# Ji4chenLi/t2v-turbo

Measured on AMD Instinct MI355X. Metric: UNet denoise steps/sec (16f 320x512 latent), higher is better.
Workload: dtype bf16; 1 GPU; VideoCrafter2 UNet forward, B=1 per GPU, latent (1,4,16,40,64), ctx (1,77,1024), 4-step LCM timestep table, random-init weights (zero-init tensors re-drawn); parallelism=replicas x1, hip_graph=True, graph_captured=True

## Files before the change

### t2v-turbo_amd/csrc/build.py

```python
import os
import subprocess
import sys

HERE = os.path.dirname(os.path.abspath(__file__))
PKG = os.path.dirname(HERE)
ROOT = os.path.dirname(PKG)
SOURCES = ["gemm.hip", "gemm_exp.hip", "gemm_fuse.hip", "conv_halo.hip", "linear_pr.hip", "norm.hip", "attention.hip", "elementwise.hip", "backward.hip", "backward_unet.hip", "train.hip", "attention_bwd.hip", "wgrad_tn.hip", "full_grad.hip", "replay.hip"]
EXPERIMENTAL = os.environ.get("T2V_EXPERIMENTAL") == "1"
if EXPERIMENTAL:
    SOURCES = SOURCES + ["gemm2.hip", "ffn.hip"]
LIB = os.path.abspath(os.environ["T2V_HIP_LIB_OUT"]) if os.environ.get("T2V_HIP_LIB_OUT") else os.path.join(PKG, "libt2v_hip_exp.so" if EXPERIMENTAL else "libt2v_hip.so")
FLAGS = ["--offload-arch=gfx950", "-O3", "-std=c++17", "-fPIC", "-Wno-unused-value",
         "-I", os.path.join(ROOT, "include"), "-I", HERE] + (["-DT2V_EXPERIMENTAL"] if EXPERIMENTAL else []) + os.environ.get("T2V_EXTRA_HIPCC_FLAGS", "").split()


def _hipcc():
    for c in (os.environ.get("HIPCC"), "/opt/rocm/bin/hipcc", "hipcc"):
        if c and (os.path.isabs(c) and os.path.exists(c) or not os.path.isabs(c)):
            return c
    return "hipcc"


def needs_build():
    if not os.path.exists(LIB):
        return True
    t = os.path.getmtime(LIB)
    deps = [os.path.join(HERE, s) for s in SOURCES] + [os.path.join(HERE, "common.h"), os.path.join(HERE, "gn_bwd_common.h"), os.path.join(HERE, "tile80.h"), os.path.join(HERE, "gemm2.h"), os.path.join(HERE, "gelu_poly.h"),
                                                        os.path.join(ROOT, "include", "t2v_hip.h")]
    return any(os.path.getmtime(d) > t for d in deps)


EXTRA_DEPS = {"gemm.hip": ["gemm2.h", "gelu_poly.h"], "gemm_exp.hip": ["gemm.hip", "gemm2.h", "gelu_poly.h"], "gemm_fuse.hip": ["gemm.hip", "gemm2.h", "gelu_poly.h"],
              "linear_pr.hip": ["gelu_poly.h"],
              "conv_halo.hip": ["tile80.h"], "gemm2.hip": ["tile80.h", "gemm2.h"], "backward.hip": ["gn_bwd_common.h"],
              "backward_unet.hip": ["gn_bwd_common.h"]}


def _stale(src, obj):
    if not os.path.exists(obj):
        return True
    t = os.path.getmtime(obj)
    deps = [os.path.join(HERE, src), os.path.join(HERE, "common.h"), os.path.join(ROOT, "include", "t2v_hip.h"), os.path.abspath(__file__)]
    deps += [os.path.join(HERE, d) for d in EXTRA_DEPS.get(src, [])]
    return any(os.path.getmtime(d) > t for d in deps)


def build(force=False, verbose=True):
    if not force and not needs_build():
        return LIB
    hipcc = _hipcc()
    objs = []
    procs = []
    for s in SOURCES:
        variant = bool(os.environ.get("T2V_HIP_LIB_OUT") or os.environ.get("T2V_EXTRA_HIPCC_FLAGS") or EXPERIMENTAL)
        o = os.path.join(HERE, s.replace(".hip", ".variant.o" if variant else ".o"))
        objs.append(o)
        if not force and not variant and not _stale(s, o):
            continue
        cmd = [hipcc] + FLAGS + ["-c", os.path.join(HERE, s), "-o", o]
        if verbose:
            print(" ".join(cmd), flush=True)
        procs.append((cmd, subprocess.Popen(cmd)))
    for cmd, p in procs:
        if p.wait() != 0:
            raise RuntimeError("hipcc failed: " + " ".join(cmd))
    cmd = [hipcc, "--offload-arch=gfx950", "-shared", "-fPIC", "-o", LIB] + objs
    if verbose:
        print(" ".join(cmd), flush=True)
    subprocess.check_call(cmd)
    return LIB


if __name__ == "__main__":
    build(force="--force" in sys.argv)
    print(LIB)
```

### t2v-turbo_amd/csrc/gemm.hip

```cpp
#include "common.h"
#ifdef T2V_EXPERIMENTAL
#include "gemm2.h"
#endif
#include "gelu_poly.h"
#include <cstdlib>
#include <type_traits>

struct GemmParams {
    t2v_gemm_desc d;
    const void* zero;
    int K, nk, taps, nsrc;
    int gh, gw;
    int kh, kw, stride, pad_y, pad_x, ups;
    int h_out, w_out;
    int tiles_m, tiles_n;
    int xcd_m, xcd_n;
    int nblk;
    int blk_start[8], blk_r0[8], blk_c0[8], blk_w[8];
    int vec4;
    int splits, nk_per_split;
    float* ws;
    int debug;
};

// ... 1009 lines not shown
}

}

int t2v_gemm_launch_experimental(int cfg, GemmParams& p, hipStream_t s);
int t2v_gemm_launch_ln(int cfg, GemmParams& p, hipStream_t s);
int t2v_gemm_launch_fused(int cfg, int fuse, GemmParams& p, hipStream_t s);
int t2v_gemm_fuse_tile(int cfg, int act, int fuse);
#ifdef T2V_GEMM_FUSE_ONLY
namespace {
template <int BM, int BN, int WM, int WN, int STAGES, int BK, int WPE>
int launch_fused(int fuse, GemmParams& p, hipStream_t s) {
    switch (fuse) {
        case 1: return launch_impl<BM, BN, WM, WN, STAGES, BK, WPE, true, false, false, 1>(p, s);
        case 2: return launch_impl<BM, BN, WM, WN, STAGES, BK, WPE, true, false, false, 2>(p, s);
        case 4: return launch_impl<BM, BN, WM, WN, STAGES, BK, WPE, true, false, false, 4>(p, s);
        case 8: return launch_impl<BM, BN, WM, WN, STAGES, BK, WPE, true, false, false, 8>(p, s);
        case 16: return launch_impl<BM, BN, WM, WN, STAGES, BK, WPE, true, false, false, 16>(p, s);
        case 18: return launch_impl<BM, BN, WM, WN, STAGES, BK, WPE, true, false, false, 18>(p, s);
        default: return T2V_EINVAL;
    }
}
}
int t2v_gemm_fuse_tile(int cfg, int act, int fuse) {
    if ((fuse == 4 || (fuse & 16)) && cfg == 19) cfg = 7;
    switch (cfg) {
        case 1: case 4: case 10: case 18: case 26: case 30: case 33: return 4;
        case 31: case 32: return act == T2V_ACT_GEGLU ? 4 : 31;
        case 6: case 7: case 13: case 16: case 19: case 25: return cfg == 19 ? 19 : (cfg == 16 ? 16 : 7);
        case 11: case 14: case 17: case 29: return cfg == 17 ? 17 : 11;
        case 12: case 15: case 20: case 21: case 24: case 27: return cfg == 20 ? 20 : 12;
        case 22: case 23: case 28: return act == T2V_ACT_GEGLU ? 17 : 23;
        case 3: case 9: return 9;
        case 2: case 5: return 5;
        default: return 0;
    }
}
int t2v_gemm_launch_fused(int cfg, int fuse, GemmParams& p, hipStream_t s) {
    switch (cfg) {
        case 4: return launch_fused<128, 128, 2, 2, 3, 64, 1>(fuse, p, s);
        case 5: return launch_fused<128, 64, 2, 2, 3, 64, 1>(fuse, p, s);
        case 7: return launch_fused<256, 128, 4, 2, 3, 64, 2>(fuse, p, s);
        case 9: return launch_fused<256, 64, 4, 2, 3, 64, 2>(fuse, p, s);
        case 11: return launch_fused<128, 256, 2, 4, 3, 64, 2>(fuse, p, s);
        case 12: return launch_fused<256, 256, 2, 4, 2, 64, 2>(fuse, p, s);
        case 16: return launch_fused<256, 128, 2, 2, 3, 32, 2>(fuse, p, s);
        case 17: return launch_fused<128, 256, 1, 4, 3, 32, 2>(fuse, p, s);
        case 19: return launch_fused<256, 128, 4, 2, 3, 32, 4>(fuse, p, s);
        case 20: return launch_fused<256, 256, 2, 4, 4, 32, 2>(fuse, p, s);
        case 23: return launch_fused<160, 320, 5, 2, 3, 32, 3>(fuse, p, s);
        case 31: return launch_fused<128, 128, 2, 4, 3, 64, 2>(fuse, p, s);
        default: return T2V_EINVAL;
    }
}
#elif defined(T2V_GEMM_EXP_ONLY)
int t2v_gemm_launch_ln(int cfg, GemmParams& p, hipStream_t s) {
    (void)cfg;
    return launch_impl<160, 320, 5, 2, 3, 32, 3, true, false, true>(p, s);
}
int t2v_gemm_launch_experimental(int cfg, GemmParams& p, hipStream_t s) {
    switch (cfg) {
        case 24: return launch<256, 256, 2, 2, 3, 32, 1>(p, s);
        case 25: return launch<256, 128, 4, 2, 2, 64, 2, true>(p, s);
        case 26: return launch<128, 128, 2, 2, 2, 64, 2, true>(p, s);
        case 27: return launch<256, 256, 2, 4, 2, 32, 2, true>(p, s);
        case 28: return launch<160, 320, 5, 2, 2, 32, 3, true>(p, s);
        case 29: return launch<128, 256, 1, 4, 2, 32, 2, true>(p, s);
        case 30: return launch<128, 128, 4, 2, 3, 64, 2>(p, s);
        case 31: return launch<128, 128, 2, 4, 3, 64, 2>(p, s);
        case 32: return launch<128, 128, 2, 4, 4, 32, 2>(p, s);
        case 33: return launch<128, 128, 4, 2, 4, 32, 2>(p, s);
        default: return T2V_EINVAL;
    }
}
#else

namespace {
struct TileCfg { int bm, bn, wtn, bk = 64; };
const TileCfg kCfg[] = {{0, 0, 0},      {128, 128, 64}, {128, 64, 32},  {256, 64, 64}, {128, 128, 64},
                        {128, 64, 32},  {256, 128, 64}, {256, 128, 64}, {64, 128, 32}, {256, 64, 32},
                        {128, 128, 64}, {128, 256, 64},
                        {256, 256, 64}, {256, 128, 64}, {128, 256, 64}, {256, 256, 64},
                        {256, 128, 64, 32}, {128, 256, 64, 32}, {128, 128, 64, 32}, {256, 128, 64, 32},
                        {256, 256, 64, 32}, {256, 256, 64, 32},
                        {160, 320, 32, 64}, {160, 320, 32, 32},
                        {256, 256, 128, 32},
                        {256, 128, 64, 64}, {128, 128, 64, 64}, {256, 256, 64, 32}, {160, 320, 32, 32}, {128, 256, 64, 32},
                        {128, 128, 64, 64}, {128, 128, 32, 64}, {128, 128, 32, 32}, {128, 128, 64, 32}};
constexpr int kNumCfg = 33;

int dispatch(int cfg, GemmParams& p, hipStream_t s) {
    switch (cfg) {
        case 1: return launch<128, 128, 2, 2, 2>(p, s);
        case 2: return launch<128, 64, 2, 2, 2>(p, s);
        case 3: return launch<256, 64, 4, 1, 2>(p, s);
        case 4: return launch<128, 128, 2, 2, 3>(p, s);
        case 5: return launch<128, 64, 2, 2, 3>(p, s);
        case 6: return launch<256, 128, 4, 2, 2>(p, s);
        case 7: return launch<256, 128, 4, 2, 3>(p, s);
        case 8: return launch<64, 128, 1, 4, 3>(p, s);
        case 9: return launch<256, 64, 4, 2, 3>(p, s);
        case 10: return launch<128, 128, 2, 2, 4>(p, s);
        case 11: return launch<128, 256, 2, 4, 3>(p, s);
        case 12: return launch<256, 256, 2, 4, 2>(p, s);
        case 13: return launch<256, 128, 2, 2, 2>(p, s);
        case 14: return launch<128, 256, 1, 4, 2>(p, s);
        case 15: return launch<256, 256, 4, 2, 2>(p, s);
        case 16: return launch<256, 128, 2, 2, 3, 32, 2>(p, s);
        case 17: return launch<128, 256, 1, 4, 3, 32, 2>(p, s);
        case 18: return launch<128, 128, 2, 2, 4, 32, 2>(p, s);
        case 19: return launch<256, 128, 4, 2, 3, 32, 4>(p, s);
        case 20: return launch<256, 256, 2, 4, 4, 32, 2>(p, s);
        case 21: return launch<256, 256, 4, 2, 4, 32, 2>(p, s);
        case 22: return launch<160, 320, 5, 2, 2, 64, 3>(p, s);
        case 23: return launch<160, 320, 5, 2, 3, 32, 3>(p, s);
        case 24: case 25: case 26: case 27: case 28: case 29: case 30: case 31: case 32: case 33:
            return t2v_gemm_launch_experimental(cfg, p, s);
        default: return T2V_EINVAL;
    }
}

}

static int g_force_cfg = 0, g_force_split = 0, g_debug = 0;
extern "C" int t2v_gemm_debug(int bits) { g_debug = bits; return T2V_OK; }
extern "C" int t2v_gemm_force_config(int cfg) { g_force_cfg = cfg; return T2V_OK; }
extern "C" int t2v_gemm_force_split(int s) { g_force_split = s; return T2V_OK; }
extern "C" int t2v_gemm_num_configs(void) { return kNumCfg; }

static int gemm_prepare(const t2v_gemm_desc* dd, GemmParams& p, int& cfg_out, int& fuse, int& fuse_cfg, bool& fuse_ok) {
    T2V_REQUIRE(dd && dd->a0 && dd->w && dd->out, T2V_EINVAL, "t2v_gemm: null pointer");
    T2V_REQUIRE(!dd->ln_in && !dd->gn_coef, T2V_EINVAL, "t2v_gemm: ln_in / gn_coef (a norm of the input rows) are t2v_linear_pr's; normalise first or ask t2v_linear_pr_supported");
    p.d = *dd;
    t2v_gemm_desc& d = p.d;
    if (!d.a1) { d.c1 = 0; d.lda1 = 0; }
    if (d.batch <= 0) d.batch = 1;
    if (d.batch_inner <= 0) d.batch_inner = 1;
    T2V_REQUIRE(d.M > 0 && d.N > 0, T2V_EINVAL, "t2v_gemm: empty problem");
    T2V_REQUIRE(d.c0 > 0 && d.c0 % 64 == 0 && d.c1 % 64 == 0, T2V_ESHAPE, "t2v_gemm: channels must be multiples of 64");
    T2V_REQUIRE(d.lda0 % 8 == 0 && d.lda1 % 8 == 0 && d.ldw % 8 == 0, T2V_ESHAPE, "t2v_gemm: lda/ldw must be multiples of 8");
    T2V_REQUIRE(((uintptr_t)d.a0 % 16 == 0) && ((uintptr_t)d.w % 16 == 0) && (!d.a1 || (uintptr_t)d.a1 % 16 == 0), T2V_ESHAPE,
                "t2v_gemm: operands must be 16-byte aligned");
    T2V_REQUIRE(d.a_stride0 % 8 == 0 && d.a_stride1 % 8 == 0 && d.w_stride0 % 8 == 0 && d.w_stride1 % 8 == 0, T2V_ESHAPE,
                "t2v_gemm: batch strides must be multiples of 8");
    T2V_REQUIRE(d.batch <= 65535, T2V_ESHAPE, "t2v_gemm: batch too large");
    if (d.drop_thr)
        T2V_REQUIRE(d.drop_seed && d.act == T2V_ACT_NONE && d.drop_ncols > 0 && d.drop_ncols % 4 == 0 && d.drop_col0 % 4 == 0 &&
                        d.drop_col0 >= 0 && d.drop_col0 + d.N <= d.drop_ncols && d.batch == 1,
                    T2V_EINVAL, "t2v_gemm: dropout epilogue (seed pointer, column geometry in multiples of 4, no activation, no batch)");
    p.nsrc = d.a1 ? 2 : 1;
    p.gh = d.h_in; p.gw = d.w_in;
    p.kh = 3; p.kw = 3; p.stride = 1; p.pad_y = 1; p.pad_x = 1; p.ups = 0;
    int n_grid = d.n_img;
    switch (d.mode) {
        case T2V_GEMM_LINEAR: p.kh = p.kw = 1; p.pad_y = p.pad_x = 0; p.gh = p.gw = 1; n_grid = d.M; break;
        case T2V_GEMM_CONV3X3: break;
        case T2V_GEMM_CONV3X3_S2: p.stride = 2; break;
        case T2V_GEMM_CONV3X3_S2_PAD01: p.stride = 2; p.pad_y = p.pad_x = 0; break;
        case T2V_GEMM_CONV3X3_UP2: p.ups = 1; break;
        case T2V_GEMM_TCONV3:
            T2V_REQUIRE(d.frames > 0 && d.n_img % d.frames == 0, T2V_EINVAL, "t2v_gemm: frames");
            p.kw = 1; p.pad_x = 0; p.gh = d.frames; p.gw = d.h_in * d.w_in; n_grid = d.n_img / d.frames;
            break;
        default: T2V_REQUIRE(false, T2V_EINVAL, "t2v_gemm: bad mode");
    }
    if (d.mode != T2V_GEMM_LINEAR) T2V_REQUIRE(d.n_img > 0 && d.h_in > 0 && d.w_in > 0, T2V_EINVAL, "t2v_gemm: conv geometry");
    p.taps = p.kh * p.kw;
    p.h_out = ((p.gh << p.ups) + 2 * p.pad_y - p.kh) / p.stride + 1;
    p.w_out = ((p.gw << p.ups) + 2 * p.pad_x - p.kw) / p.stride + 1;
    if (d.mode == T2V_GEMM_CONV3X3_S2_PAD01) {
        p.h_out = (p.gh + 1 - 3) / 2 + 1; p.w_out = (p.gw + 1 - 3) / 2 + 1;
    }
    T2V_REQUIRE((long long)d.M == (long long)n_grid * p.h_out * p.w_out, T2V_EINVAL, "t2v_gemm: M does not match the geometry");
    p.K = p.taps * (d.c0 + d.c1);
    p.nk = p.K / 64;
    T2V_REQUIRE(d.ldw >= p.K, T2V_EINVAL, "t2v_gemm: ldw < K");
    if (d.act == T2V_ACT_GEGLU) T2V_REQUIRE(d.N % 128 == 0, T2V_ESHAPE, "t2v_gemm: GEGLU needs N % 128 == 0");
    if (d.rowvec) T2V_REQUIRE(d.rowvec_div > 0, T2V_EINVAL, "t2v_gemm: rowvec_div");
    p.zero = t2v_zero_page();
    T2V_REQUIRE(p.zero, T2V_EHIP, "t2v_gemm: zero page allocation failed");
    const int n_out = d.act == T2V_ACT_GEGLU ? d.N / 2 : d.N;
    p.vec4 = (d.ldo % 8 == 0) && (n_out % 4 == 0) && ((uintptr_t)d.out % 16 == 0) && (d.o_stride0 % 8 == 0) &&
             (d.o_stride1 % 8 == 0) && (!d.residual || (d.ldr % 8 == 0 && (uintptr_t)d.residual % 16 == 0)) &&
             (!d.bias || (uintptr_t)d.bias % 16 == 0) && (!d.rowvec || ((uintptr_t)d.rowvec % 16 == 0 && d.ld_rowvec % 4 == 0));
    if (d.act == T2V_ACT_GEGLU) T2V_REQUIRE(p.vec4, T2V_ESHAPE, "t2v_gemm: GEGLU needs 8-byte aligned rows");

    int cfg = g_force_cfg ? g_force_cfg : d.tile_cfg;
    if (cfg < 0 || cfg > kNumCfg) cfg = 0;
    if (cfg == 0) {
        if (d.N % 128 == 0 || d.N >= 1024) cfg = (d.M >= 8192 && p.nk >= 8) ? 7 : 4;
        else if (d.M >= 8192 && d.N % 64 == 0) cfg = 9;
        else cfg = 5;
    }
    if (d.act == T2V_ACT_GEGLU && kCfg[cfg].wtn < 64) cfg = 4;
    p.nk = p.K / kCfg[cfg].bk;
    int splits = g_force_split ? g_force_split : d.split_k;
    const long long tiles = (long long)((d.M + kCfg[cfg].bm - 1) / kCfg[cfg].bm) * ((d.N + kCfg[cfg].bn - 1) / kCfg[cfg].bn) * d.batch;
    const bool can_split = d.ws && d.act != T2V_ACT_GEGLU && d.N % 4 == 0 && p.vec4;
    if (splits <= 0) {
        splits = 1;
        if (can_split && tiles < 160 && p.K / 64 >= 16) {
            splits = (int)((448 + tiles - 1) / tiles);
            if (splits > p.K / 512) splits = p.K / 512;
            if (splits > 16) splits = 16;
        }
    }
    if (!can_split) splits = 1;
    if (splits > 1 && (long long)splits * d.batch * d.M * d.N * 4 > d.ws_bytes) {
        splits = (int)(d.ws_bytes / ((long long)d.batch * d.M * d.N * 4));
        if (splits < 2) splits = 1;
    }
    if (splits > p.nk) splits = p.nk;
    p.nk_per_split = (p.nk + splits - 1) / splits;
    splits = (p.nk + p.nk_per_split - 1) / p.nk_per_split;
    p.splits = splits;
    p.ws = (float*)d.ws;
    p.debug = g_debug;
    cfg_out = cfg;
    fuse = (d.rowstat_out ? 1 : 0) | (d.colstat_out ? 2 : 0) | (d.lnf_stats ? 4 : 0) | (d.lora_t ? 16 : 0);
    static const bool fast_dropout = !(getenv("T2V_GEMM_FAST_DROPOUT") && getenv("T2V_GEMM_FAST_DROPOUT")[0] == '0');
    const bool auto_drop = !fuse && !d.lora_t && d.drop_thr && fast_dropout && !d.rowvec && d.act == T2V_ACT_NONE && !d.ln_out && d.batch == 1;
    if (auto_drop) fuse = 8;
    fuse_cfg = 0;
    fuse_ok = false;
    if (fuse) {
        T2V_REQUIRE(fuse == 1 || fuse == 2 || fuse == 4 || fuse == 8 || fuse == 16 || fuse == 18, T2V_EINVAL,
                    "t2v_gemm: one of rowstat_out / colstat_out / lnf_stats per launch (lora_t alone or with colstat_out)");
        if (fuse & 16)
            T2V_REQUIRE(d.lora_u && d.lora_n_leaf > 0 && d.lora_n_leaf % 32 == 0 && d.N % d.lora_n_leaf == 0 && d.ld_lora_t % 8 == 0 &&
                            d.ld_lora_u % 8 == 0 && d.ld_lora_u >= 64 && d.ld_lora_t >= 64 * (d.N / d.lora_n_leaf) &&
                            (uintptr_t)d.lora_t % 16 == 0 && (uintptr_t)d.lora_u % 16 == 0 && d.act == T2V_ACT_NONE &&
                            (!d.drop_thr || (d.drop_seed && d.drop_ncols % 4 == 0 && d.drop_col0 % 4 == 0)),
                        T2V_ESHAPE, "t2v_gemm: lora_t: rank-64 rows [M][64 leaves], lora_u [N][64], N a multiple of lora_n_leaf (% 32), no activation");
        T2V_REQUIRE(!d.ln_out && d.batch == 1, T2V_EINVAL, "t2v_gemm: fused statistics: no batch, no LayerNorm second output");
        if (fuse == 1)
            T2V_REQUIRE(d.N % 32 == 0 && d.ld_rowstat >= d.N / 16 && d.ld_rowstat % 4 == 0 && (uintptr_t)d.rowstat_out % 16 == 0 &&
                            d.act == T2V_ACT_NONE, T2V_ESHAPE, "t2v_gemm: rowstat_out needs N % 32 == 0, ld_rowstat >= N / 16 (% 4), no activation");
        if (fuse & 2)
            T2V_REQUIRE(d.M % 32 == 0 && d.N % 2 == 0 && (uintptr_t)d.colstat_out % 16 == 0 && d.act != T2V_ACT_GEGLU, T2V_ESHAPE,
                        "t2v_gemm: colstat_out needs M % 32 == 0");
        if (fuse == 4)
            T2V_REQUIRE(d.mode == T2V_GEMM_LINEAR && !d.a1 && d.lnf_s && d.bias && d.lnf_nblk > 0 && d.lnf_nblk % 2 == 0 && d.lnf_nblk <= 40 &&
                            d.c0 == 32 * d.lnf_nblk && d.lnf_ld >= 2 * d.lnf_nblk && d.lnf_ld % 4 == 0 && (uintptr_t)d.lnf_stats % 16 == 0 &&
                            (uintptr_t)d.lnf_s % 16 == 0 && !d.residual && !d.rowvec && !d.drop_thr && d.act != T2V_ACT_SILU,
                        T2V_ESHAPE, "t2v_gemm: lnf_stats: LINEAR over C = 32 lnf_nblk <= 1280 channels, lnf_s and bias given, no residual / "
                                    "row vector / dropout");
        fuse_cfg = t2v_gemm_fuse_tile(cfg, d.act, fuse);
        fuse_ok = fuse_cfg != 0 && p.splits == 1 && gemm_is_fast(p, fuse == 8 || (fuse & 16) != 0) && !(d.act == T2V_ACT_GEGLU && kCfg[fuse_cfg].wtn < 64);
        if ((fuse & 16) && fuse_cfg != 0 && d.N != d.lora_n_leaf) {
            const int wtn = fuse_cfg == 23 ? 160 : kCfg[fuse_cfg].wtn;
            for (int s = 0; s < d.N && fuse_ok; s += wtn)
                if ((s + wtn - 1 < d.N ? s + wtn - 1 : d.N - 1) / d.lora_n_leaf - s / d.lora_n_leaf > 1) fuse_ok = false;
        }
        if (fuse == 8 && !(fuse_cfg == cfg || cfg == 28 || cfg == 32)) fuse_ok = false;
        if (fuse_ok) { p.nk = p.K / kCfg[fuse_cfg].bk; p.nk_per_split = p.nk; }
        if (fuse == 8 && !fuse_ok) fuse = 0;
        return T2V_OK;
    }
    return T2V_OK;
}

#ifdef T2V_EXPERIMENTAL
static int g_gemm2 = -1;
extern "C" int t2v_gemm2_enable(int on) { g_gemm2 = on ? 1 : 0; return T2V_OK; }
static int gemm2_route(const t2v_gemm_desc* dd, int fuse, Gemm2Params& p2, int& c2) {
    c2 = 0;
    if (g_gemm2 < 0) g_gemm2 = (getenv("T2V_GEMM2") && getenv("T2V_GEMM2")[0] == '1') ? 1 : 0;
    const int want = g_force_cfg ? g_force_cfg : dd->tile_cfg;
    const int forced = (want == 50 || want == 51) ? want - 49 : 0;
    if ((fuse & ~2) || dd->ln_out || !(forced || (g_gemm2 && !g_force_cfg))) return T2V_OK;
    return t2v_gemm2_prepare(dd, p2, forced, c2);
}
#endif

extern "C" int t2v_gemm_fuse_supported(const t2v_gemm_desc* dd) {
    GemmParams p;
    int cfg = 0, fuse = 0, fuse_cfg = 0;
    bool ok = false;
    const int rc = gemm_prepare(dd, p, cfg, fuse, fuse_cfg, ok);
    if (rc != T2V_OK) return rc;
#ifdef T2V_EXPERIMENTAL
    if (fuse == 2) {
        Gemm2Params p2;
        int c2 = 0;
        const int rc2 = gemm2_route(dd, fuse, p2, c2);
        if (rc2 != T2V_OK) return rc2;
        if (c2) return 1;
    }
#endif
    return ((fuse & ~8) && ok) ? 1 : 0;
}

extern "C" int t2v_gemm_plan(const t2v_gemm_desc* dd, int* tile_cfg, int* splits) {
    GemmParams p;
    int cfg = 0, fuse = 0, fuse_cfg = 0;
    bool ok = false;
    const int rc = gemm_prepare(dd, p, cfg, fuse, fuse_cfg, ok);
    if (rc != T2V_OK) return rc;
    if (tile_cfg) *tile_cfg = (fuse && ok) ? fuse_cfg : cfg;
    if (splits) *splits = p.splits;
    return T2V_OK;
}

extern "C" int t2v_gemm(const t2v_gemm_desc* dd, void* stream) {
    GemmParams p;
    int cfg = 0, fuse = 0, fuse_cfg = 0;
    bool fuse_ok = false;
    const int rc = gemm_prepare(dd, p, cfg, fuse, fuse_cfg, fuse_ok);
    if (rc != T2V_OK) return rc;
    t2v_gemm_desc& d = p.d;
    hipStream_t s = (hipStream_t)stream;
#ifdef T2V_EXPERIMENTAL
    {
        Gemm2Params p2;
        int c2 = 0;
        const int rc2 = gemm2_route(dd, fuse, p2, c2);
        if (rc2 != T2V_OK) return rc2;
        if (c2) return t2v_gemm2_dispatch(c2, p2, s);
    }
#endif
    if (fuse) {
        T2V_REQUIRE(fuse_ok, T2V_ESHAPE, "t2v_gemm: this launch cannot carry fused statistics (ask t2v_gemm_fuse_supported first)");
        return t2v_gemm_launch_fused(fuse_cfg, fuse, p, s);
    }
    if (d.ln_out) {
        cfg = 23;
        p.nk = p.K / kCfg[cfg].bk;
        p.splits = 1; p.nk_per_split = p.nk;
        const bool fast = p.vec4 && d.N % 16 == 0 && d.alpha == 1.0f && !d.out_f32 && !d.drop_thr &&
                          (!d.rowvec || ((uintptr_t)d.rowvec % 16 == 0 && d.ld_rowvec % 4 == 0));
        T2V_REQUIRE(d.N == 320 && d.batch == 1 && d.act == T2V_ACT_NONE && fast && d.ln_gamma && d.ln_beta && d.ld_ln_out % 8 == 0 &&
                        (uintptr_t)d.ln_out % 16 == 0 && (uintptr_t)d.ln_gamma % 16 == 0 && (uintptr_t)d.ln_beta % 16 == 0,
                    T2V_ESHAPE, "t2v_gemm: the LayerNorm output needs N == 320, bf16 out, alpha 1, aligned operands, no batch / activation");
        return t2v_gemm_launch_ln(cfg, p, s);
    }
    return dispatch(cfg, p, s);
}
#endif
```

Measured before the change: 48.03 steps/s.

## Add split-K small-M GEMM kernel with intra-block wave reduction

```diff
diff --git a/t2v-turbo_amd/csrc/build.py b/t2v-turbo_amd/csrc/build.py
--- a/t2v-turbo_amd/csrc/build.py
+++ b/t2v-turbo_amd/csrc/build.py
@@ -5,7 +5,7 @@
 HERE = os.path.dirname(os.path.abspath(__file__))
 PKG = os.path.dirname(HERE)
 ROOT = os.path.dirname(PKG)
-SOURCES = ["gemm.hip", "gemm_exp.hip", "gemm_fuse.hip", "conv_halo.hip", "linear_pr.hip", "norm.hip", "attention.hip", "elementwise.hip", "backward.hip", "backward_unet.hip", "train.hip", "attention_bwd.hip", "wgrad_tn.hip", "full_grad.hip", "replay.hip"]
+SOURCES = ["gemm.hip", "gemm_exp.hip", "gemm_fuse.hip", "conv_halo.hip", "linear_pr.hip", "gemm_small_m.hip", "norm.hip", "attention.hip", "elementwise.hip", "backward.hip", "backward_unet.hip", "train.hip", "attention_bwd.hip", "wgrad_tn.hip", "full_grad.hip", "replay.hip"]
 EXPERIMENTAL = os.environ.get("T2V_EXPERIMENTAL") == "1"
 if EXPERIMENTAL:
     SOURCES = SOURCES + ["gemm2.hip", "ffn.hip"]
@@ -31,7 +31,7 @@
 
 
 EXTRA_DEPS = {"gemm.hip": ["gemm2.h", "gelu_poly.h"], "gemm_exp.hip": ["gemm.hip", "gemm2.h", "gelu_poly.h"], "gemm_fuse.hip": ["gemm.hip", "gemm2.h", "gelu_poly.h"],
-              "linear_pr.hip": ["gelu_poly.h"],
+              "linear_pr.hip": ["gelu_poly.h"], "gemm_small_m.hip": ["gelu_poly.h"],
               "conv_halo.hip": ["tile80.h"], "gemm2.hip": ["tile80.h", "gemm2.h"], "backward.hip": ["gn_bwd_common.h"],
               "backward_unet.hip": ["gn_bwd_common.h"]}
 
diff --git a/t2v-turbo_amd/csrc/gemm.hip b/t2v-turbo_amd/csrc/gemm.hip
--- a/t2v-turbo_amd/csrc/gemm.hip
+++ b/t2v-turbo_amd/csrc/gemm.hip
@@ -1335,6 +1335,32 @@
     return T2V_OK;
 }
 
+#ifdef T2V_HOSTSIM
+#define T2V_SMALL_M_SYM __attribute__((weak))
+#else
+#define T2V_SMALL_M_SYM
+#endif
+T2V_SMALL_M_SYM int t2v_gemm_small_m_enabled();
+T2V_SMALL_M_SYM bool t2v_gemm_small_m_gate(const t2v_gemm_desc& d);
+T2V_SMALL_M_SYM bool t2v_gemm_small_m_takes(const t2v_gemm_desc& d, int vec4);
+T2V_SMALL_M_SYM int t2v_gemm_small_m_launch(const t2v_gemm_desc& d, const void* zero, int taps, int gh, int gw, int kw, int pad_y, int pad_x, int h_out,
+                                            int w_out, hipStream_t s);
+static bool small_m_route(const t2v_gemm_desc* dd, const GemmParams& p, int fuse) {
+#ifdef T2V_HOSTSIM
+    if (!&t2v_gemm_small_m_launch) return false;
+#endif
+    const int mode = t2v_gemm_small_m_enabled();
+    return !g_force_cfg && dd->tile_cfg == 0 && !fuse && mode && t2v_gemm_small_m_takes(p.d, p.vec4) && (mode == 2 || t2v_gemm_small_m_gate(p.d));
+}
+extern "C" int t2v_gemm_small_m_supported(const t2v_gemm_desc* dd) {
+    GemmParams p;
+    int cfg = 0, fuse = 0, fuse_cfg = 0;
+    bool ok = false;
+    const int rc = gemm_prepare(dd, p, cfg, fuse, fuse_cfg, ok);
+    if (rc != T2V_OK) return rc;
+    return small_m_route(dd, p, fuse) ? 1 : 0;
+}
+
 extern "C" int t2v_gemm(const t2v_gemm_desc* dd, void* stream) {
     GemmParams p;
     int cfg = 0, fuse = 0, fuse_cfg = 0;
@@ -1343,6 +1369,8 @@
     if (rc != T2V_OK) return rc;
     t2v_gemm_desc& d = p.d;
     hipStream_t s = (hipStream_t)stream;
+    if (small_m_route(dd, p, fuse))
+        return t2v_gemm_small_m_launch(d, p.zero, p.taps, p.gh, p.gw, p.kw, p.pad_y, p.pad_x, p.h_out, p.w_out, s);
 #ifdef T2V_EXPERIMENTAL
     {
         Gemm2Params p2;
diff --git a/t2v-turbo_amd/csrc/gemm_small_m.hip b/t2v-turbo_amd/csrc/gemm_small_m.hip
--- /dev/null
+++ b/t2v-turbo_amd/csrc/gemm_small_m.hip
@@ -0,0 +1,271 @@
+#include "common.h"
+#include "gelu_poly.h"
+#include <cstdlib>
+#include <type_traits>
+
+struct SmallMParams {
+    t2v_gemm_desc d;
+    const void* zero;
+    int C, ngroups;
+    int gh, gw, kw, pad_y, pad_x, h_out, w_out;
+    int tiles_m;
+};
+
+namespace {
+
+constexpr int kSmWaves = 8;
+constexpr int kSmRing = 8;
+constexpr int kSmPitch = 68;
+constexpr int kSmPlane = 64 * kSmPitch;
+constexpr int kSmSmem = kSmWaves * kSmPlane * 4;
+
+template <int I, int N, class F>
+__device__ __forceinline__ void sm_static_for(F&& f) {
+    if constexpr (I < N) {
+        f(std::integral_constant<int, I>{});
+        sm_static_for<I + 1, N>(f);
+    }
+}
+
+template <bool CONV, bool GEGLU>
+__global__ __launch_bounds__(kSmWaves * 64) __attribute__((amdgpu_waves_per_eu(2, 2))) void gemm_small_m_kernel(const SmallMParams p) {
+    constexpr int R = kSmRing;
+    extern __shared__ __attribute__((aligned(16))) char smem[];
+    const t2v_gemm_desc& d = p.d;
+    const int tid = threadIdx.x, lane = tid & 63;
+    const int wave = __builtin_amdgcn_readfirstlane(tid >> 6);
+    const int l31 = lane & 31, hi = lane >> 5;
+    const int tile = xcd_contiguous(blockIdx.x, gridDim.x);
+    const int tile_n = tile / p.tiles_m, tile_m = tile - tile_n * p.tiles_m;
+    const int m0 = tile_m * 64, n0 = tile_n * 64;
+    const int g_begin = wave * p.ngroups / kSmWaves, ngw = (wave + 1) * p.ngroups / kSmWaves - g_begin;
+
+    const bf16_t* wp[2];
+#pragma unroll
+    for (int b = 0; b < 2; ++b) wp[b] = (const bf16_t*)d.w + (long long)(n0 + 32 * b + l31) * d.ldw + (long long)g_begin * 64 + 32 * hi;
+    const bf16_t* const zero = (const bf16_t*)p.zero;
+    const bf16_t* const abase = (const bf16_t*)d.a0 + 32 * hi;
+    const bf16_t* ap[2];
+    int ainc[2];
+    int an[2], ay[2], ax[2];
+    int ltap = 0, lc = 0;
+#pragma unroll
+    for (int i = 0; i < 2; ++i) {
+        const int m = m0 + 32 * i + l31;
+        if constexpr (CONV) {
+            const int hw_o = p.h_out * p.w_out;
+            const int n = m / hw_o, rem = m - n * hw_o;
+            ay[i] = rem / p.w_out; ax[i] = rem - ay[i] * p.w_out;
+            an[i] = m < d.M ? n : -1;
+            ap[i] = zero; ainc[i] = 0;
+        } else {
+            an[i] = ay[i] = ax[i] = 0;
+            if (m < d.M) { ap[i] = abase + (long long)m * d.lda0 + (long long)g_begin * 64; ainc[i] = 64; }
+            else { ap[i] = zero; ainc[i] = 0; }
+        }
+    }
+    if constexpr (CONV) {
+        const int k0 = g_begin * 64;
+        ltap = k0 / p.C; lc = k0 - ltap * p.C;
+    }
+
+    bf16x8_t ra[R][2], rw[R][2];
+    f32x16_t acc[2][2];
+#pragma unroll
+    for (int i = 0; i < 2; ++i)
+#pragma unroll
+        for (int b = 0; b < 2; ++b)
+#pragma unroll
+            for (int e = 0; e < 16; ++e) acc[i][b][e] = 0.f;
+
+    const bf16_t* src[2] = {zero, zero};
+    auto load_step = [&](auto slot_tag, auto j_tag) {
+        constexpr int S = decltype(slot_tag)::value, J = decltype(j_tag)::value;
+        if constexpr (J == 0) {
+            if constexpr (CONV) {
+                const int ky = p.kw == 1 ? ltap : ltap / 3, kx = ltap - ky * p.kw;
+#pragma unroll
+                for (int i = 0; i < 2; ++i) {
+                    const int uy = ay[i] + ky - p.pad_y, ux = ax[i] + kx - p.pad_x;
+                    const bool ok = an[i] >= 0 && uy >= 0 && uy < p.gh && ux >= 0 && ux < p.gw;
+                    const long long row = ((long long)an[i] * p.gh + uy) * p.gw + ux;
+                    src[i] = ok ? abase + row * d.lda0 + lc : zero;
+                }
+                lc += 64;
+                if (lc == p.C) { lc = 0; ++ltap; }
+            } else {
+#pragma unroll
+                for (int i = 0; i < 2; ++i) { src[i] = ap[i]; ap[i] += ainc[i]; }
+            }
+        }
+#pragma unroll
+        for (int b = 0; b < 2; ++b) rw[S][b] = *(const bf16x8_t*)(wp[b] + 8 * J);
+#pragma unroll
+        for (int i = 0; i < 2; ++i) ra[S][i] = *(const bf16x8_t*)(src[i] + 8 * J);
+        if constexpr (J == 3) {
+#pragma unroll
+            for (int b = 0; b < 2; ++b) wp[b] += 64;
+        }
+    };
+    auto compute = [&](auto slot_tag) {
+        constexpr int S = decltype(slot_tag)::value;
+#pragma unroll
+        for (int i = 0; i < 2; ++i)
+#pragma unroll
+            for (int b = 0; b < 2; ++b)
+                acc[i][b] = __builtin_amdgcn_mfma_f32_32x32x16_bf16(rw[S][b], ra[S][i], acc[i][b], 0, 0, 0);
+    };
+
+    const int nst = 4 * ngw;
+    sm_static_for<0, R - 1>([&](auto s) {
+        constexpr int S = decltype(s)::value;
+        if (S < nst) load_step(s, std::integral_constant<int, S & 3>{});
+    });
+#pragma unroll 1
+    for (int base = 0; base < nst; base += R) {
+        sm_static_for<0, R>([&](auto u) {
+            constexpr int U = decltype(u)::value, L = (U + R - 1) % R;
+            const int st = base + U;
+            if (st < nst) {
+                if (st + R - 1 < nst) load_step(std::integral_constant<int, L>{}, std::integral_constant<int, L & 3>{});
+                __builtin_amdgcn_sched_barrier(0);
+                compute(u);
+                __builtin_amdgcn_sched_barrier(0);
+            }
+        });
+    }
+
+    float* const sf = (float*)smem;
+    {
+        float* pl = sf + wave * kSmPlane + l31 * kSmPitch + 4 * hi;
+#pragma unroll
+        for (int i = 0; i < 2; ++i)
+#pragma unroll
+            for (int b = 0; b < 2; ++b)
+#pragma unroll
+                for (int r = 0; r < 4; ++r)
+                    *(float4*)(pl + 32 * i * kSmPitch + 32 * b + 8 * r) =
+                        make_float4(acc[i][b][4 * r], acc[i][b][4 * r + 1], acc[i][b][4 * r + 2], acc[i][b][4 * r + 3]);
+    }
+    __syncthreads();
+
+    const int row = tid >> 3, cc = tid & 7;
+    const int gm = m0 + row;
+    constexpr int NV = GEGLU ? 4 : 8;
+    const int col_a = GEGLU ? 4 * cc : 8 * cc, col_b = GEGLU ? 32 + 4 * cc : 8 * cc + 4;
+    float va[4] = {0.f, 0.f, 0.f, 0.f}, vb[4] = {0.f, 0.f, 0.f, 0.f};
+#pragma unroll
+    for (int s = 0; s < kSmWaves; ++s) {
+        const float* pl = sf + s * kSmPlane + row * kSmPitch;
+        const float4 ta = *(const float4*)(pl + col_a), tb = *(const float4*)(pl + col_b);
+        va[0] += ta.x; va[1] += ta.y; va[2] += ta.z; va[3] += ta.w;
+        vb[0] += tb.x; vb[1] += tb.y; vb[2] += tb.z; vb[3] += tb.w;
+    }
+    if (gm >= d.M) return;
+    float v[NV];
+    int ch_out;
+    if constexpr (GEGLU) {
+        float4 ba = make_float4(0.f, 0.f, 0.f, 0.f), bb = ba;
+        if (d.bias) { ba = *(const float4*)(d.bias + n0 + col_a); bb = *(const float4*)(d.bias + n0 + col_b); }
+        v[0] = (va[0] + ba.x) * fast_gelu(vb[0] + bb.x);
+        v[1] = (va[1] + ba.y) * fast_gelu(vb[1] + bb.y);
+        v[2] = (va[2] + ba.z) * fast_gelu(vb[2] + bb.z);
+        v[3] = (va[3] + ba.w) * fast_gelu(vb[3] + bb.w);
+        ch_out = n0 / 2 + 4 * cc;
+    } else {
+#pragma unroll
+        for (int e = 0; e < 4; ++e) { v[e] = va[e]; v[4 + e] = vb[e]; }
+        ch_out = n0 + 8 * cc;
+        if (d.bias) {
+#pragma unroll
+            for (int q = 0; q < 2; ++q) {
+                const float4 t = *(const float4*)(d.bias + ch_out + 4 * q);
+                v[4 * q] += t.x; v[4 * q + 1] += t.y; v[4 * q + 2] += t.z; v[4 * q + 3] += t.w;
+            }
+        }
+    }
+    if (d.rowvec) {
+        const float* rv = d.rowvec + (long long)(gm / d.rowvec_div) * d.ld_rowvec + ch_out;
+#pragma unroll
+        for (int q = 0; q < NV / 4; ++q) {
+            const float4 t = *(const float4*)(rv + 4 * q);
+            v[4 * q] += t.x; v[4 * q + 1] += t.y; v[4 * q + 2] += t.z; v[4 * q + 3] += t.w;
+        }
+    }
+    if (d.residual) {
+        const bf16_t* rp = (const bf16_t*)d.residual + (long long)gm * d.ldr + ch_out;
+        if constexpr (GEGLU) {
+            const uint2 t = *(const uint2*)rp;
+            v[0] += __uint_as_float(t.x << 16); v[1] += __uint_as_float(t.x & 0xffff0000u);
+            v[2] += __uint_as_float(t.y << 16); v[3] += __uint_as_float(t.y & 0xffff0000u);
+        } else {
+            float rf[8];
+            unpack8(*(const uint4*)rp, rf);
+#pragma unroll
+            for (int e = 0; e < 8; ++e) v[e] += rf[e];
+        }
+    }
+    if (d.act == T2V_ACT_SILU) {
+#pragma unroll
+        for (int e = 0; e < NV; ++e) v[e] = silu_f(v[e]);
+    }
+    bf16_t* op = (bf16_t*)d.out + (long long)gm * d.ldo + ch_out;
+    if constexpr (GEGLU) {
+        uint2 o;
+        o.x = pack2bf(v[0], v[1]); o.y = pack2bf(v[2], v[3]);
+        *(uint2*)op = o;
+    } else {
+        *(uint4*)op = pack8(v);
+    }
+}
+
+template <bool CONV, bool GEGLU>
+int sm_launch(const SmallMParams& p, int tiles, hipStream_t s) {
+    static bool attr_set = false;
+    if (!attr_set) {
+        hipFuncSetAttribute((const void*)gemm_small_m_kernel<CONV, GEGLU>, hipFuncAttributeMaxDynamicSharedMemorySize, kSmSmem);
+        attr_set = true;
+    }
+    hipLaunchKernelGGL((gemm_small_m_kernel<CONV, GEGLU>), dim3(tiles), dim3(kSmWaves * 64), kSmSmem, s, p);
+    T2V_CHECK_LAUNCH();
+    return T2V_OK;
+}
+
+}
+
+static int g_small_m_mode = -1;
+extern "C" int t2v_gemm_small_m_mode(int mode) { g_small_m_mode = mode; return T2V_OK; }
+int t2v_gemm_small_m_enabled() {
+    static const int env = getenv("T2V_GEMM_SMALL_M") ? atoi(getenv("T2V_GEMM_SMALL_M")) : 1;
+    const int m = g_small_m_mode >= 0 ? g_small_m_mode : env;
+    return m < 0 ? 0 : (m > 2 ? 2 : m);
+}
+bool t2v_gemm_small_m_gate(const t2v_gemm_desc& d) {
+    return d.mode == T2V_GEMM_LINEAR && d.N == 64 && d.c0 >= 1024 && d.c0 <= 1280;
+}
+
+bool t2v_gemm_small_m_takes(const t2v_gemm_desc& d, int vec4) {
+    if (d.mode != T2V_GEMM_LINEAR && d.mode != T2V_GEMM_TCONV3 && d.mode != T2V_GEMM_CONV3X3) return false;
+    if (d.a1 || d.c1 || d.batch > 1 || d.alpha != 1.0f || d.out_f32 || d.drop_thr || d.ln_out || d.rowstat_out || d.colstat_out || d.lnf_stats ||
+        d.lora_t)
+        return false;
+    if (d.act != T2V_ACT_NONE && d.act != T2V_ACT_GEGLU && d.act != T2V_ACT_SILU) return false;
+    if (d.M > 640 || d.N % 64 || d.c0 % 64 || !vec4) return false;
+    if (d.act == T2V_ACT_GEGLU && (d.ldo % 4 || (d.residual && d.ldr % 4))) return false;
+    return true;
+}
+
+int t2v_gemm_small_m_launch(const t2v_gemm_desc& d, const void* zero, int taps, int gh, int gw, int kw, int pad_y, int pad_x, int h_out, int w_out,
+                            hipStream_t s) {
+    SmallMParams p;
+    p.d = d;
+    p.zero = zero;
+    p.C = d.c0;
+    p.ngroups = taps * d.c0 / 64;
+    p.gh = gh; p.gw = gw; p.kw = kw; p.pad_y = pad_y; p.pad_x = pad_x; p.h_out = h_out; p.w_out = w_out;
+    p.tiles_m = (d.M + 63) / 64;
+    const int tiles = p.tiles_m * (d.N / 64);
+    const bool geglu = d.act == T2V_ACT_GEGLU;
+    if (taps > 1) return geglu ? sm_launch<true, true>(p, tiles, s) : sm_launch<true, false>(p, tiles, s);
+    return geglu ? sm_launch<false, true>(p, tiles, s) : sm_launch<false, false>(p, tiles, s);
+}
```

New measurement: 47.98 steps/s. No clear change (-0.1%).
